# saga0619/libdwbc

Hardware: AMD Instinct MI355X
Metric: HQP control cycles/sec (batched TOCABI) (higher is better)
Workload: dtype f64; 1 GPU; BASELINE configs[1]: batch=1024 per GPU, TOCABI double support, 2-level HQP (pelvis 6D + upper-body rotation), tau limit 300, fp64; batch_per_gpu=1024, threads_per_instance=128, lds_bytes_per_instance=39152, collective_backend=none (one rank)

## Files before the change

__graft_entry__.py:

```python
import os
import subprocess
import sys

ROOT = os.path.dirname(os.path.abspath(__file__))
if ROOT not in sys.path:
    sys.path.insert(0, ROOT)


def build():
    env = dict(os.environ)
    env.setdefault("PYTORCH_ROCM_ARCH", "gfx950")
    csrc = os.path.join(ROOT, "libdwbc_amd", "csrc")
    import signal

    packs = [subprocess.Popen(["make", "-C", csrc, "pack", f"N={n}", f"NB={nb}", "ARCH=gfx950"], env=env, start_new_session=True)
             for n, nb in ((37, 32), (23, 18), (43, 38))]
    done = False
    try:
        subprocess.check_call(["make", "-C", csrc, "ARCH=gfx950"], env=env)
        subprocess.check_call(["make", "-C", os.path.join(ROOT, "oracle")], env=env)
        subprocess.check_call(["make", "-C", os.path.join(ROOT, "tests", "qp_probe"), "gpu", "ARCH=gfx950"], env=env)
        subprocess.check_call(["make", "-C", os.path.join(ROOT, "tests", "wave_probe"), "gpu", "ARCH=gfx950"], env=env)
        import libdwbc_amd
        from libdwbc_amd import _lib

        _lib.load()
        import tempfile

        from tests import cases

        with tempfile.TemporaryDirectory() as tmp:
            libdwbc_amd.build_pack(libdwbc_amd.Model.from_urdf(cases.variant_urdf(os.path.join(tmp, "fh.urdf"), cases.HEAD_JOINTS)), tree=True)
        for p in packs:
            if p.wait() != 0:
                raise subprocess.CalledProcessError(p.returncode, p.args)
        done = True
    finally:
        if not done:
            for p in packs:
                if p.poll() is None:
                    try:
                        os.killpg(p.pid, signal.SIGTERM)
                    except ProcessLookupError:
                        pass
            for p in packs:
                try:
                    p.wait(timeout=30)
                except subprocess.TimeoutExpired:
                    try:
                        os.killpg(p.pid, signal.SIGKILL)
                    except ProcessLookupError:
                        pass
                    p.wait()


def smoke():
    import numpy as np

    import libdwbc_amd as D
    from oracle import orc
    from tests import cases

    B = 16
    model = D.Model.from_urdf(cases.URDF)
    wbc = D.Batch(model, B, device=0)
    for c in cases.CONTACTS_2:
        wbc.add_contact(c["link"], c["point"], c["lx"], c["ly"], c["mu"], c["muz"])
    wbc.add_task(0, D.TASK_LINK_6D, 0)
    wbc.add_task(1, D.TASK_LINK_ROTATION, 15)
    wbc.set_torque_limit(np.array(cases.TAU_LIM))
    q, flags, fstar = cases.synth_batch(B, seed=7)
    wbc.set_state(q)
    wbc.set_contact(flags)
    wbc.set_fstar_all(fstar)
    wbc.solve()
    tau = wbc.get("tau")
    status = wbc.get("status")
    M = orc.make_model(cases.tocabi_model())
    S = orc.make_setup(cases.CONTACTS_2, cases.TASKS_2LEVEL, cases.TAU_LIM)
    tau_ref, wr_ref, st_ref, _ = orc.cycle_batch(M, S, q, flags, fstar, 1)
    err = float(np.abs(tau - tau_ref).max())
    assert (status == st_ref).all(), (status, st_ref)
    assert err < 1e-6, err
    print(f"smoke ok: B={B} max|tau - oracle| = {err:.3e}")


if __name__ == "__main__":
    build()
    if len(sys.argv) > 1 and sys.argv[1] == "smoke":
        smoke()
```

libdwbc_amd/csrc/dwbc_cycle2p.h:

```cpp
#pragma once
#include "dwbc_cycle2.h"

namespace dwbc {

template <int N, int NB, int NLV>
struct Lds4 {
    static constexpr bool compact = true;
    static constexpr bool batch_reads = true;
    static constexpr int M = N - 6;
    static constexpr int C = 6 * kMaxActiveContacts;
    static constexpr int K = C - 6;
    static constexpr int T = kMaxTaskDof;
    static constexpr int WLD = 32;
    static constexpr int max2(int a, int b) { return a > b ? a : b; }
    static constexpr int ev(int a) { return (a + 1) & ~1; }
    static constexpr int tg = 0;
    static constexpr int tt = tg + M;
    static constexpr int tc = tt + M;
    static constexpr int PC = tc + M;
    static constexpr int Rc = PC + C;
    static constexpr int Pc = Rc + kMaxActiveContacts * 9;
    static constexpr int fs = Pc + kMaxActiveContacts * 3;
    static constexpr int flg = fs + kMaxLevels * kMaxTaskDof;
    static constexpr int q = ev(flg + 4);
// ... 24 lines not shown
    static constexpr int c_Vb = Jtt + max2(NLV * N * T, C * N);
    static constexpr int c_VG = c_Vb + M * K;
    static constexpr int hs = c_VG + M * K;
    static constexpr int hs_size = 4 * 36 + 72;
    static constexpr int ms = hs + hs_size;
    static constexpr int c_s1 = ms;
    static constexpr int c_s2 = ms + max2(C * K, 64);
    static constexpr int c_Lam = c_s2;
    static constexpr int ms_size = max2(C * K, 64) + C * C;
    static constexpr int kin = ms + ms_size;
    static constexpr int k_Iw = kin;
    static constexpr int k_Ic = k_Iw + NB * 10;
    static constexpr int k_Rl = k_Iw + NB * 3;
    static constexpr int k_anc = k_Ic + NB * 10 - 2 * NB;
    static_assert(k_Rl + NB * 9 <= k_anc, "local rotations must not reach the ancestor indices");
    static constexpr int k_S = k_Ic + NB * 10;
    static constexpr int k_F = k_S + N * 6;
    static constexpr int kin_end = k_F + N * 6;
    static constexpr bool a_overlay = false, a_packed = true;
    static constexpr int k_A = U;
    static_assert(N * (N + 1) / 2 <= (UAend - U), "the staged mass matrix borrows the U / T1x-sized region");
    static constexpr int c_Y = kin;
    static constexpr int c_D = kin + C * N;
    static constexpr int c_BJ = c_D + (NLV * T + 1) * C;
    static constexpr int T1x = ev(max2(c_BJ + NLV * T * T, kin + 2 * T * M + 6 * T * T + 3 * T));
    static_assert(T1x + NLV * T * MS <= kin_end, "Y, D, the task Gram blocks and T1x borrow the phase-1a scratch");
    static constexpr int p4_dl = kin;
    static constexpr int p4_e = p4_dl + ev(NVS * C);
    static constexpr int p4_w = p4_e + C * VS;
    static constexpr int p4_ts = U;
    static constexpr int p4_cv = p4_ts + M * VS;
    static_assert(kin % 2 == 0 && U % 2 == 0, "16-byte aligned rows of the phase-4 blocks (lds_rows_axpy)");
    static_assert(p4_w + K * VS <= c_D, "phase-4 scratch stays below D and the task Gram blocks (the helper reads them in parallel)");
    static_assert(p4_cv + 6 * VS <= UAend, "torques and base residuals borrow the place of the staged mass matrix");
    static constexpr int c_QW = kin;
    static constexpr int c_QWp = c_QW + T * M;
    static constexpr int c_Pi = c_QWp + T * M;
    static constexpr int c_Z = c_Pi + T * T;
    static constexpr int c_s2b = c_Z + T * T;
    static constexpr int cod_Q = c_s2b + T * T, cod_v = cod_Q + T * T, cod_G = cod_v + 3 * T, cod_T = cod_G + T * T;
    static_assert(cod_T + T * T <= T1x, "slow-route scratch stays below T1x");
    static constexpr int xl(int lv) { return U; }
    static constexpr int t_base = Rw;
    static constexpr int wm = ev(t_base + NLV * 6);
    static constexpr int t_fv = wm + C * WLD;
    static constexpr int qp_V = t_fv + C;
    static constexpr int p5_end = qp_V + kQpLd;
    static_assert(p5_end <= fend, "QP scratch over the link frames");
    static constexpr int c_T1 = 0;
    static constexpr int total = kin_end;
    static constexpr int total_bytes = total * (int)sizeof(real_t) + 64;
    static constexpr int FNl = NwJw, comp = flg, Jcm = 0, Pt = 0, c_Gi = 0, T1r = T1x, c_Q = T1x, c_Jt = Jtt, t_F = wm, t_s1 = wm, jk = 0;
};

#if defined(DWBC_HOST_EMU)
#define DWBC_PAIR_BARRIER(i) ((void)0)
#elif defined(DWBC_STAGE_TIMERS)
#define DWBC_PAIR_BARRIER(i)                                                                      \
    do {                                                                                          \
        if (diag && th.tid == 0) diag[(is_main ? DG_TIME : DG_FTIME) + (i)] = (int)(clock64() - t_start_); \
        __syncthreads();                                                                          \
        if (diag && th.tid == 0 && is_main) diag[DG_FTIME + 8 + (i)] = (int)(clock64() - t_start_); \
    } while (0)
#else
#define DWBC_PAIR_BARRIER(i) __syncthreads()
#endif
#if defined(DWBC_HOST_EMU)
#define DWBC_PAIR_BARRIER_X() ((void)0)
#else
#define DWBC_PAIR_BARRIER_X() __syncthreads()
#endif
#if defined(DWBC_STAGE_TIMERS) && !defined(DWBC_HOST_EMU)
#define DWBC_PSTAMP(i) do { DWBC_SYNC(); if (diag && th.tid == 0) diag[DG_FTIME + (i)] = (int)(clock64() - t_start_); } while (0)
#ifndef DWBC_PMASK
#define DWBC_PMASK 0ull
#endif
#define DWBC_PSTAMP_M(i) do { if constexpr (((DWBC_PMASK) >> ((i) - 41)) & 1ull) DWBC_PSTAMP(i); } while (0)
#else
#define DWBC_PSTAMP(i) ((void)0)
#define DWBC_PSTAMP_M(i) ((void)0)
#endif

template <int MR, int NCV, int KV, bool SYNC_STORE, class FA, class FB, class FS, class FC>
DWBC_WDEV void wave_gemm(FA fa, FB fb, FS fstore, FC fc) {
    constexpr int MT = (MR + 15) / 16, KB = (KV + 3) / 4;
    static_assert(NCV <= 16, "one column tile");
#if !defined(DWBC_HOST_EMU)
    static_assert(sizeof(real_t) == 8, "fp64 build");
    typedef double g_d4 __attribute__((ext_vector_type(4)));
    const int lane = (int)(threadIdx.x & 63u), li = lane & 15, lk = lane >> 4;
    const int jc = (NCV < 16 && li >= NCV) ? NCV - 1 : li;
    double av[MT][KB], bv[KB];
    static_for<0, KB>([&](auto sc) {
        constexpr int s_ = decltype(sc)::value;
        constexpr bool kwhole = 4 * s_ + 3 < KV;
        const int kk = kwhole ? 4 * s_ + lk : (4 * s_ + lk < KV ? 4 * s_ + lk : KV - 1);
        const bool kin = kwhole || 4 * s_ + lk < KV;
        const double b_ = fb(sc, kk, jc);
        bv[s_] = kin ? b_ : 0.0;
        static_for<0, MT>([&](auto tc) {
            constexpr int t = decltype(tc)::value;
            constexpr bool rwhole = 16 * t + 15 < MR;
            const int ic = rwhole ? 16 * t + li : (16 * t + li < MR ? 16 * t + li : MR - 1);
            const double a_ = fa(tc, sc, ic, kk);
            av[t][s_] = kin ? a_ : 0.0;
        });
    });
    g_d4 acc[MT];
#pragma unroll
    for (int t = 0; t < MT; t++)
#pragma unroll
        for (int r = 0; r < 4; r++) {
            const int i = 16 * t + lk + 4 * r;
            acc[t][r] = fc(i < MR ? i : MR - 1, jc);
        }
#pragma unroll
    for (int s_ = 0; s_ < KB; s_++)
#pragma unroll
        for (int t = 0; t < MT; t++) acc[t] = __builtin_amdgcn_mfma_f64_16x16x4f64(av[t][s_], bv[s_], acc[t], 0, 0, 0);
    if (SYNC_STORE) DWBC_SYNC();
#pragma unroll
    for (int t = 0; t < MT; t++)
#pragma unroll
        for (int r = 0; r < 4; r++) {
            const int i = 16 * t + lk + 4 * r;
            if (i < MR && li < NCV) fstore(i, li, acc[t][r]);
        }
#else
    real_t tmp[MR][NCV];
    for (int i = 0; i < MR; i++)
        for (int j = 0; j < NCV; j++) tmp[i][j] = fc(i, j);
    static_for<0, KB>([&](auto sc) {
        constexpr int s_ = decltype(sc)::value;
        static_for<0, MT>([&](auto tc) {
            constexpr int t = decltype(tc)::value;
            for (int li = 0; li < 16; li++)
                for (int lk = 0; lk < 4; lk++) {
                    const int i = 16 * t + li, kk = 4 * s_ + lk;
                    if (i >= MR || kk >= KV) continue;
                    const real_t a_ = fa(tc, sc, i, kk);
                    for (int j = 0; j < NCV; j++) tmp[i][j] += a_ * fb(sc, kk, j);
                }
        });
    });
    for (int i = 0; i < MR; i++)
        for (int j = 0; j < NCV; j++) fstore(i, j, tmp[i][j]);
#endif
}
template <int MR, int NCV, int KV, bool SYNC_STORE, class FA, class FB, class FS>
DWBC_WDEV void wave_gemm(FA fa, FB fb, FS fstore) {
    wave_gemm<MR, NCV, KV, SYNC_STORE>(fa, fb, fstore, [](int, int) { return real_t(0.0); });
}

template <class R>
DWBC_WDEV int spd_inverse12_lds(R *Mx, R *Out, R *scl) {
#if defined(DWBC_HOST_EMU)
    return spd_inverse_small(Mx, 12, 12, Out, 12, scl);
#else
    static_assert(sizeof(R) == 8, "fp64 build");
    const int lane = (int)(threadIdx.x & 63u);
    DWBC_SYNC();
    double s[12], dg, dsc;
    {
        const int col = lane < 12 ? lane : 0;
        const double a = Mx[col * 12 + col];
        int e2 = 0;
        (void)frexp(a > 0.0 ? a : 1.0, &e2);
        dsc = (lane < 12 && a > 0.0) ? ldexp(1.0, -(e2 >> 1)) : 1.0;
        if (lane < 12) scl[lane] = dsc;
    }
    DWBC_SYNC();
    {
        const int col = lane < 12 ? lane : 0;
#pragma unroll
        for (int i = 0; i < 12; i++) {
            const double v_ = Mx[i * 12 + col] * scl[i] * dsc;
            s[i] = lane < 12 ? v_ : 0.0;
        }
        const double d_ = Mx[col * 12 + col] * dsc * dsc;
        dg = lane < 12 ? d_ : 1.0;
    }
    DWBC_SYNC();
    int ok = 1;
    {
        DWBC_LANE_OPAQUE(lp);
#pragma unroll
        for (int i = 0; i < 12; i++) s[i] = (i == lp) ? dg - 1.0 : s[i];
    }
    double dg2 = dg - 2.0;
    lds_pivot<12, 11, 0>(s, dg2, ok, (unsigned)(size_t)Mx, lane);
    ok = DWBC_FLAG_UNIFORM(ok);
    DWBC_SYNC();
    if (lane < 12) {
        DWBC_LANE_OPAQUE(le);
#pragma unroll
        for (int i = 0; i < 12; i++) {
            const double v_ = (i == le) ? -dg2 : -s[i];
            Out[i * 12 + lane] = v_ * scl[i] * dsc;
        }
    }
    DWBC_SYNC();
    return ok;
#endif
}

template <int N, int NB, int NLV, int NT, class Topo>
DWBC_DEV void cycle_instance_v2p(int wave, Thr th, const Setup &su, const BatchIO &io, int inst, real_t *L) {
    using S = Lds4<N, NB, NLV>;
    constexpr int M = S::M, C = S::C, T = S::T;
    constexpr bool kTree = !std::is_same<Topo, TopoGeneric>::value;
    static_assert(kTree, "the paired kernel is built for a constant kinematic tree");
    static_assert(kMaxActiveContacts == 2, "two 6D contacts");
    static_assert(N + 1 <= 64 && NB <= 64 && NT >= 1, "one q entry and one body per lane (request phase, *_lane forms of dwbc_front.h)");
    DWBC_LANE_DECL;
    const bool is_main = wave <= 0, is_help = wave != 0;
    const int nb = NB;
    const real_t *body = io.body;
    const int *topo = io.topo;
    const io_t *qin = io.q + (size_t)inst * (N + 1);
    int *diag = io.diag ? io.diag + (size_t)inst * DG_COUNT : nullptr;
    DWBC_STAMP_INIT();
    const int npair = topo[3 * nb];
    PLA(real_t, b_rec, kBodyStride);
    PL(int, b_par);
    PL(int, b_len);
    real_t q_base[7] = {0, 0, 0, 0, 0, 0, 0};
    PL(real_t, q_cp);
    PL(real_t, q_jt);
    LANES { LV(q_cp) = real_t(0.0); LV(q_jt) = real_t(0.0); LV(b_par) = 0; }
    int pairw[kCrbaPairRounds<N, NT>];
    if (is_main) {
        LANES {
            LV(q_cp) = (real_t)qin[lane < N + 1 ? lane : 0];
            LV(q_jt) = (real_t)qin[(lane >= 1 && lane < NB) ? 5 + lane : 0];
        }
        for (int a = 0; a < 6; a++) q_base[a] = (real_t)qin[a];
        q_base[6] = (real_t)qin[N];
        lane_record_fetch<NB, BF_RT, BF_MASS>(body, b_rec);
        LANES { LV(b_par) = topo[lane < NB ? lane : 0]; }
#pragma unroll
        for (int r = 0; r < kCrbaPairRounds<N, NT>; r++) pairw[r] = topo[3 * nb + 1 + (r * NT + th.tid < npair ? r * NT + th.tid : npair - 1)];
    }
    static_assert(kMaxLevels * kMaxTaskDof <= 64, "one f* entry per lane");
    PL(real_t, fs_req);
    LANES { LV(fs_req) = real_t(0.0); }
    if (is_help) {
        const io_t *fin = io.fstar + (size_t)inst * su.fstar_total;
        LANES {
            if (lane < su.fstar_total) LV(fs_req) = (real_t)fin[lane];
        }
    }
    const unsigned char *fl = io.flags + (size_t)inst * su.n_contacts;
    int flb[kMaxContacts];
    int lane_zero = 0;
    DWBC_FLAG_VGPR(lane_zero);
#pragma unroll
    for (int i = 0; i < kMaxContacts; i++) flb[i] = (i < su.n_contacts ? fl + i : (const unsigned char *)topo)[lane_zero];
    lane_record_fetch<NB, BF_MASS, kBodyStride>(body, b_rec);
    LANES { LV(b_len) = topo[2 * NB + (lane < NB ? lane : 0)]; }
    real_t *JCt = L + S::c_JC, *Yt = L + S::c_Y, *Lam = L + S::c_Lam, *JbT = L + S::JbT, *Vb = L + S::c_Vb, *VG = L + S::c_VG;
    real_t *flg = L + S::flg;

    PLA(real_t, s, N);
    PL(real_t, dg);
    int st_contact = 1;

    real_t *Rw = L + S::Rw, *pw = L + S::pw, *aw = L + S::aw, *Rl = L + S::k_Rl;
    real_t *Iw = L + S::k_Iw, *Icm = L + S::k_Ic, *Sm = L + S::k_S, *Fm = L + S::k_F;
    if (is_main) {
        LANES {
            if (lane < N + 1) L[S::q + lane] = LV(q_cp);
        }
        for (int i = th.tid; i < 3 * M; i += NT) L[S::tg + i] = real_t(0.0);
        DWBC_PSTAMP_M(56);
        constexpr int kRounds = jump_rounds(Topo::maxdepth);
        PLA(real_t, Ri, 9);
        PLA(real_t, pi, 3);
        PL(real_t, an);
        joint_transforms_lane<NB>(q_base, q_jt, b_rec, b_par, kRounds, Rw, pw, Rl, Iw, L + S::k_anc, Ri, pi, an);
        DWBC_PSTAMP_M(57);
        world_transforms_jump_lane<NB>(kRounds, Rw, pw, Rl, Iw, L + S::k_anc, Ri, pi, an);
        DWBC_PSTAMP_M(58);
        world_axes_lane<NB>(b_rec, Ri, aw);
        DWBC_PSTAMP_M(59);
    }
    if (is_help) {
        LANES {
            if (lane < su.fstar_total) L[S::fs + lane] = LV(fs_req);
        }
        if (th.tid == 0) { flg[0] = real_t(1.0); flg[1] = real_t(0.0); }
    }
    int act_c[kMaxActiveContacts] = {0, 0};
    int nc = 0, nflag = 0;
#pragma unroll
    for (int i = 0; i < kMaxContacts; i++) {
        if (i < su.n_contacts) {
            const int f_ = DWBC_FLAG_UNIFORM(flb[i]);
            if (f_ && nc < kMaxActiveContacts) act_c[nc++] = i;
            nflag += f_ ? 1 : 0;
        }
    }
    if (is_main) DWBC_PSTAMP_M(55);
    const bool too_many = nflag > kMaxActiveContacts;
    const int cd = 6 * nc, k = cd > 6 ? cd - 6 : 0;
    DWBC_PAIR_BARRIER(0);

    if (is_main) {
        world_inertias_lane<NB>(b_rec, Rw, pw, Iw);
        DWBC_SYNC();
        DWBC_PSTAMP_M(51);
        composite_inertias_scan_lane<0, 5>(b_len, nb, Iw, Icm);
        DWBC_SYNC();
    }
    if (is_help) {
        world_inertias_lane<NB>(b_rec, Rw, pw, Iw);
        DWBC_SYNC();
        composite_inertias_scan_lane<5, 10>(b_len, nb, Iw, Icm);
        DWBC_SYNC();
    }
    if (is_main) {
        motion_axes<N, NT>(th, Rw, pw, aw, Sm);
        DWBC_SYNC();
    }
    DWBC_PAIR_BARRIER_X();
    if (is_main) {
        DWBC_PSTAMP_M(52);
        body_forces<N, NT>(th, Icm, Sm, Fm);
        DWBC_SYNC();
        DWBC_PSTAMP_M(53);
        real_t *A = L + S::k_A;
        for (int idx = th.tid; idx < N * (N + 1) / 2; idx += NT) A[idx] = real_t(0.0);
        DWBC_SYNC();
        crba_pairs_fill<N, NT>(th, npair, pairw, Sm, Fm, A);
        DWBC_SYNC();
        DWBC_PSTAMP_M(54);
        load_mass_columns<N>(A, s, dg, L + S::G);
        DWBC_PSTAMP_M(41);
    }
    if (is_help) {
        for (int a = 0; a < nc; a++) {
            const int ci = act_c[a], link = su.c_link[ci];
            const real_t *R = Rw + link * 9;
            for (int r = th.tid; r < 12; r += NT) {
// ... 737 lines not shown
```

libdwbc_amd/csrc/dwbc_qp_wave.h:

```cpp
#pragma once
#include <type_traits>

#include "dwbc_wave.h"

namespace dwbc {

constexpr int kQpN = 12;

template <int QN>
struct QpRowsT {
    PLA(real_t, g, QN);
    PL(real_t, hi);
    PL(real_t, lo);
    PL(int, id_hi);
    PL(int, id_lo);
};
using QpRows = QpRowsT<kQpN>;

template <int QN>
struct QpResultT {
    int status, iters, nact;
    real_t viol;
    real_t x[QN];
    int act[QN];
#if defined(DWBC_STAGE_TIMERS) && !defined(DWBC_HOST_EMU)
    long long tm[10];
#endif
};
using QpResult = QpResultT<kQpN>;

#if defined(DWBC_STAGE_TIMERS) && !defined(DWBC_HOST_EMU)
#define DWBC_QPT_INIT() long long qpt_last_ = clock64(); for (int i_ = 0; i_ < 10; i_++) out.tm[i_] = 0
#define DWBC_QPT(i) do { const long long now_ = clock64(); out.tm[i] += now_ - qpt_last_; qpt_last_ = now_; } while (0)
#else
#define DWBC_QPT_INIT() ((void)0)
#define DWBC_QPT(i) ((void)0)
#endif

#ifdef DWBC_QP_TRACE
#ifdef DWBC_HOST_EMU
#define QP_TRACE(...) printf(__VA_ARGS__)
#else
#define QP_TRACE(...) do { if (threadIdx.x == 0) printf(__VA_ARGS__); } while (0)
#endif
#endif
#define DWBC_QP_INF (dwbc::kF32 ? dwbc::real_t(1.0e30) : dwbc::real_t(1.0e300))



template <int WS, int NV = kQpN, int QN = kQpN, int KCV = (QN > 12 ? QN - 6 : 6)>
DWBC_WDEV void qp_solve_wave(QpRowsT<QN> &R, int nv, int t, int max_iter, QpResultT<QN> &out, real_t *V , const int *warm,
                             real_t vtol, PL_REF(real_t, sfin)) {
    DWBC_LANE_DECL;
    static_assert(NV <= QN && NV <= 24, "variable count");
    constexpr int SB = NV > 16 ? 32 : 16;
    const int k = nv - t;
    PLA(real_t, Mx, NV);
    PL(real_t, d);
    PL(real_t, fs);
    PL(real_t, gnv);
    PL(real_t, u);
    PL(int, akey);
    PL(real_t, ehi);
    PL(real_t, elo);
    PL(bool, rok);
    PL(int, slotbit);
    PL(real_t, val);
    PL(int, key);
    PL(real_t, m);
    PL(real_t, dz);
    PL(real_t, xl);
    DWBC_QPT_INIT();
    LANES {
        LV(xl) = real_t(0.0);
        DWBC_LANE_OPAQUE(lq);
        real_t s2 = real_t(0.0), a2 = real_t(0.0);
#pragma unroll
        for (int j = 0; j < NV; j++) {
            const real_t g2 = LV(R.g)[j] * LV(R.g)[j];
            s2 += g2;
            a2 += (j < t) ? g2 : g2 * (real_t(1.0) / (kQpScaleGI * kQpScaleGI));
        }
        const bool zrow = s2 < kQpZeroRow * kQpZeroRow;
        const real_t gn = zrow ? real_t(1.0) : sqrt(s2);
        const real_t rg = zrow ? real_t(0.0) : real_t(1.0) / gn;
        LV(fs) = zrow ? real_t(1.0) : gn / sqrt(a2);
        LV(gnv) = gn;
#pragma unroll
        for (int j = 0; j < NV; j++) {
            LV(R.g)[j] *= rg;
            LV(Mx)[j] = (lq == j) ? real_t(1.0) : real_t(0.0);
        }
        if (LV(R.hi) < DWBC_QP_INF && !zrow) LV(R.hi) *= rg;
        if (LV(R.lo) < DWBC_QP_INF && !zrow) LV(R.lo) *= rg;
        LV(ehi) = LV(R.hi) >= DWBC_QP_INF ? DWBC_QP_INF : LV(R.hi);
        LV(elo) = LV(R.lo) >= DWBC_QP_INF ? DWBC_QP_INF : LV(R.lo);
        LV(d) = real_t(0.0);
        LV(u) = real_t(0.0);
        LV(akey) = 0;
        LV(slotbit) = (lane >= SB && lane < SB + NV) ? (1 << (lane - SB)) : 0;
        LV(m) = real_t(0.0);
        LV(dz) = real_t(0.0);
    }
    DWBC_QPT(6);
    int used = 0, q = 0, it = 0, status = 1, p = 0, side = 0, kmin = 0;
    bool pick = true;
    real_t up = real_t(0.0), worst = real_t(0.0);
    real_t sp = real_t(0.0);
    int wid[QN], wpos = QN;
    if (WS && warm) {
#pragma unroll
        for (int a = 0; a < QN; a++) wid[a] = warm[a];
        wpos = 0;
    }
    for (;;) {
        bool got = false;
        if (WS && pick) {
            while (wpos < QN && !got) {
                int id = -1;
#pragma unroll
                for (int a = 0; a < QN; a++) id = (a == wpos) ? wid[a] : id;
                wpos++;
                if (id < 0) continue;
                LANES {
                    const bool mh = LV(R.id_hi) == id && LV(ehi) < DWBC_QP_INF;
                    const bool ml = LV(R.id_lo) == id && LV(elo) < DWBC_QP_INF;
                    LV(val) = mh ? LV(ehi) - LV(d) : (ml ? LV(elo) + LV(d) : DWBC_QP_INF);
                    LV(key) = (lane << 1) | (ml ? 1 : 0);
                }
                int pl;
                WAVE_ARGMIN_F32(val, pl);
                worst = BCAST(val, pl);
                kmin = BCASTI(key, pl);
                if (worst < -vtol) got = true;
            }
            if (got) {
                p = kmin >> 1;
                side = kmin & 1;
                up = real_t(0.0);
                sp = worst;
                pick = false;
            }
        }
        if (pick) {
            LANES {
                const real_t sh = LV(ehi) - LV(d);
                const real_t sl = LV(elo) + LV(d);
                const bool lo_side = sl < sh;
                LV(val) = lo_side ? sl : sh;
                LV(key) = (lane << 1) | (lo_side ? 1 : 0);
            }
            int pl;
            WAVE_ARGMIN_F32(val, pl);
            worst = BCAST(val, pl);
            kmin = BCASTI(key, pl);
            DWBC_QPT(1);
            if (!(worst < -vtol)) break;
            p = kmin >> 1;
            side = kmin & 1;
            up = real_t(0.0);
            sp = worst;
            pick = false;
        }
        if (++it > max_iter) { status = 0; break; }
        real_t gp[NV];
#pragma unroll
        for (int j = 0; j < NV; j++) gp[j] = BCASTA(R.g, j, p);
        const real_t sgn = side ? real_t(1.0) : -real_t(1.0);
        LANES {
            real_t s_ = real_t(0.0);
#pragma unroll
            for (int j = 0; j < NV; j++) s_ += LV(Mx)[j] * gp[j];
            LV(m) = sgn * s_;
        }
        real_t zu[NV];
#pragma unroll
        for (int i = 0; i < NV; i++) zu[i] = BCAST(m, i);
        LANES {
            real_t s_ = real_t(0.0);
#pragma unroll
            for (int j = 0; j < NV; j++) s_ += LV(R.g)[j] * zu[j];
            LV(dz) = s_;
        }
        real_t zg = sgn * BCAST(dz, p);
        if (zg < kQpReorth) {
            LANES {
                real_t s_ = real_t(0.0);
#pragma unroll
                for (int j = 0; j < NV; j++) s_ += LV(Mx)[j] * zu[j];
                if (lane < NV) LV(m) = s_;
            }
#pragma unroll
            for (int i = 0; i < NV; i++) zu[i] = BCAST(m, i);
            LANES {
                real_t s_ = real_t(0.0);
#pragma unroll
                for (int j = 0; j < NV; j++) s_ += LV(R.g)[j] * zu[j];
                LV(dz) = s_;
            }
            zg = sgn * BCAST(dz, p);
        }
        const bool zok = zg > (kF32 ? real_t(1e-10) : real_t(1e-20)) && q < nv;
        DWBC_QPT(2);
        LANES { LV(rok) = (LV(slotbit) & used) && LV(m) > (kF32 ? real_t(1e-6) : real_t(1e-12)); }
        real_t t1 = DWBC_QP_INF;
        int l = SB;
        bool rany;
        WAVE_ANY(rok, rany);
        if (rany) {
            LANES {
                LV(val) = LV(rok) ? LV(u) * fast_rcp(LV(m)) : DWBC_QP_INF;
                LV(key) = lane;
            }
            if constexpr (SB == 16) {
                WAVE_ARGMIN_ROW1(val, key, t1, l);
            } else {
                WAVE_ARGMIN(val, key, t1, l);
            }
        }
        const real_t t2 = zok ? -sp * fast_rcp(zg) : DWBC_QP_INF;
        const real_t tstep = t1 < t2 ? t1 : t2;
        if (!(tstep < DWBC_QP_INF)) { status = 0; break; }
        const bool full = zok && t2 <= t1;
        if (zok) {
            LANES {
                LV(d) += tstep * LV(dz);
                LV(xl) += tstep * LV(m);
            }
        }
        LANES { LV(u) -= tstep * LV(m); }
        up += tstep;
        DWBC_QPT(3);
        if (full) {
            const int slot = __builtin_ctz(~(unsigned)used);
            const real_t inv_ = fast_rcp(zg);
            LANES {
                real_t coef = LV(m) * inv_;
                if (lane == SB + slot) { coef = -inv_; LV(u) = up; LV(akey) = kmin; }
#pragma unroll
                for (int j = 0; j < NV; j++) LV(Mx)[j] -= coef * zu[j];
                LV(ehi) = ((lane << 1) == kmin) ? DWBC_QP_INF : LV(ehi);
                LV(elo) = (((lane << 1) | 1) == kmin) ? DWBC_QP_INF : LV(elo);
            }
            used |= 1 << slot;
            q++;
            pick = true;
        } else {
            const int kl = BCASTI(akey, l);
            WSYNC();
            LANES {
                if (lane == l) {
#pragma unroll
                    for (int j = 0; j < NV; j++) V[j] = LV(Mx)[j];
                }
            }
            WSYNC();
            real_t rho[NV], rr = real_t(0.0);
#pragma unroll
            for (int j = 0; j < NV; j++) { rho[j] = V[j]; rr += rho[j] * rho[j]; }
            const real_t inv_ = fast_rcp(rr);
            LANES {
                real_t dd = real_t(0.0);
#pragma unroll
                for (int j = 0; j < NV; j++) dd += LV(Mx)[j] * rho[j];
                real_t coef = dd * inv_;
                if (lane < NV) coef = -V[lane] * inv_;
#pragma unroll
                for (int j = 0; j < NV; j++) LV(Mx)[j] = (lane == l) ? real_t(0.0) : LV(Mx)[j] - coef * rho[j];
                if (lane == l) LV(u) = real_t(0.0);
                LV(ehi) = ((lane << 1) == kl) ? LV(R.hi) : LV(ehi);
                LV(elo) = (((lane << 1) | 1) == kl) ? LV(R.lo) : LV(elo);
            }
            WSYNC();
            used &= ~(1 << (l - SB));
            q--;
            LANES { LV(val) = side ? LV(R.lo) + LV(d) : LV(R.hi) - LV(d); }
            sp = BCAST(val, p);
        }
        DWBC_QPT(4);
    }
    DWBC_QPT(0);
    out.iters = it;
    out.nact = q;
    out.status = status;
    out.viol = worst >= DWBC_QP_INF ? real_t(0.0) : worst;
#pragma unroll
    for (int a = 0; a < QN; a++) {
        if (WS) {
            const int ka = BCASTI(akey, SB + a);
            const int ow = ka >> 1;
            const int idh = BCASTI(R.id_hi, ow), idl = BCASTI(R.id_lo, ow);
            out.act[a] = ((used >> a) & 1) ? ((ka & 1) ? idl : idh) : -1;
        } else {
            out.act[a] = -1;
        }
    }
#pragma unroll
    for (int i = 0; i < QN; i++) out.x[i] = real_t(0.0);
    auto final_slack = [&](int which) {
        LANES {
            const real_t gx = which == 0 ? real_t(0.0) : (which == 1 ? LV(d) : LV(dz));
            const real_t sh = LV(R.hi) >= DWBC_QP_INF ? DWBC_QP_INF : (LV(R.hi) - gx) * LV(gnv);
            const real_t sl = LV(R.lo) >= DWBC_QP_INF ? DWBC_QP_INF : (LV(R.lo) + gx) * LV(gnv);
            LV(sfin) = sl < sh ? sl : sh;
        }
    };
    if (!status || q == 0) { final_slack(0); return; }
    real_t xu[NV];
#pragma unroll
    for (int i = 0; i < NV; i++) xu[i] = BCAST(xl, i);
#pragma unroll
    for (int j = 0; j < QN; j++) out.x[j] = (j < nv) ? xu[j < NV ? j : 0] * ((j >= t) ? kQpScaleGI : real_t(1.0)) : real_t(0.0);
    if (!(k > 0 && t > 0)) { final_slack(1); return; }
    {
        real_t xs[NV];
        constexpr int KC = KCV;
        constexpr int kCgMax = KC > kQpRefine ? 4 * KC : kQpRefine;
        static_assert(NV >= KC, "variable blocks");
        bool settled = false;
        auto lex_point = [&](auto std_tag) {
            constexpr bool STD = decltype(std_tag)::value;
            real_t cx[KC], cr[KC], cp[KC], cb[KC];
#pragma unroll
            for (int i = 0; i < KC; i++) {
                real_t v = real_t(0.0);
                if constexpr (STD) {
                    v = xu[NV - KC + i];
                } else {
#pragma unroll
                    for (int j = 0; j < NV; j++) v = (j == t + i && i < k) ? xu[j] : v;
                }
                cb[i] = v;
                cx[i] = v;
            }
            auto hmul = [&](const real_t (&v)[KC]) {
                LANES {
                    real_t s_ = real_t(0.0);
                    if constexpr (STD) {
#pragma unroll
                        for (int i = 0; i < KC; i++) s_ += LV(Mx)[NV - KC + i] * v[i];
                    } else {
#pragma unroll
                        for (int j = 0; j < NV; j++) {
                            real_t vj = real_t(0.0);
#pragma unroll
                            for (int i = 0; i < KC; i++) vj = (j == t + i && i < k) ? v[i] : vj;
                            s_ += LV(Mx)[j] * vj;
                        }
                    }
                    LV(m) = s_;
                }
            };
            auto hcc = [&](int i) -> real_t {
                real_t h_;
                if constexpr (STD) h_ = BCAST(m, NV - KC + i);
                else h_ = (i < k) ? BCAST(m, t + i) : real_t(0.0);
                return h_;
            };
            hmul(cx);
            real_t rs = real_t(0.0), bn = real_t(0.0);
#pragma unroll
            for (int i = 0; i < KC; i++) {
                cr[i] = cb[i] - (cx[i] - hcc(i));
                cp[i] = cr[i];
                rs += cr[i] * cr[i];
                bn += cb[i] * cb[i];
            }
            const real_t rtol2 = kQpRefineTol * kQpRefineTol * bn;
            bool nulldir = false;
            const real_t atol2 = kQpNullRes * kQpNullRes * bn;
            for (int r = 0; r < kCgMax && rs > rtol2; r++) {
#ifdef DWBC_QP_TRACE
                QP_TRACE("  cg %d rs %.3e\n", r, (double)rs);
#endif
                hmul(cp);
                real_t ap[KC], pap = real_t(0.0), pp = real_t(0.0);
#pragma unroll
                for (int i = 0; i < KC; i++) {
                    ap[i] = cp[i] - hcc(i);
                    pap += cp[i] * ap[i];
                    pp += cp[i] * cp[i];
                }
                if (!(pap > kQpNullDir * pp)) { nulldir = true; break; }
                const real_t al = rs * fast_rcp(pap);
                real_t rs2 = real_t(0.0);
#pragma unroll
                for (int i = 0; i < KC; i++) {
                    const real_t rn = cr[i] - al * ap[i];
                    rs2 += rn * rn;
                }
                if (rs2 > rs && !(rs > atol2)) { nulldir = true; break; }
#pragma unroll
                for (int i = 0; i < KC; i++) {
                    cx[i] += al * cp[i];
                    cr[i] -= al * ap[i];
                }
// ... 58 lines not shown
```

libdwbc_amd/csrc/dwbc_wave.h:

```cpp
#pragma once
#include <math.h>

#include "dwbc_types.h"

#ifdef DWBC_HOST_EMU
#define PL(type, x) type x[64]
#define PLA(type, x, n) type x[64][n]
#define LV(x) x[lane]
#define LANES for (int lane = 0; lane < 64; ++lane)
#define WSYNC() ((void)0)
#define DWBC_LANE_DECL ((void)0)
#define DWBC_LANE_OPAQUE(name) const int name = lane
#define DWBC_LANE_OPAQUE_IF(name, cond) const int name = lane
#define DWBC_FLAG_VGPR(f) ((void)0)
#define DWBC_FLAG_UNIFORM(f) (f)
#define BCAST(x, src) ((x)[(src)])
#define BCASTA(x, j, src) ((x)[(src)][(j)])
#define SHFLA(x, j, src) ((x)[(src)][(j)])
#define SHFL(x, src) ((x)[(src)])
#define DWBC_WDEV inline
#define PLA_REF(type, name, n) type (&name)[64][n]
#define PL_REF(type, name) type (&name)[64]
#else
#define PL(type, x) type x
// ... 149 lines not shown
    do {                                                                                           \
        out_b = false;                                                                             \
        for (int l_ = 0; l_ < 64; l_++) out_b = out_b || (flag)[l_];                               \
    } while (0)
#define WAVE_ARGMIN_ROW1(val, key, out_v, out_k)                                                   \
    do {                                                                                           \
        out_v = (val)[16];                                                                         \
        out_k = (key)[16];                                                                         \
        for (int l_ = 17; l_ < 32; l_++)                                                           \
            if ((val)[l_] < out_v || ((val)[l_] == out_v && (key)[l_] < out_k)) { out_v = (val)[l_]; out_k = (key)[l_]; } \
    } while (0)
#else
namespace dwbc {
__device__ __forceinline__ unsigned long long wave_min_u64(unsigned long long x) {
#define DWBC_DPP_STEP(ctrl, rmask)                                                                         \
    {                                                                                                      \
        const int lo_ = (int)(unsigned)(x & 0xffffffffull), hi_ = (int)(unsigned)(x >> 32);                \
        const int olo_ = __builtin_amdgcn_update_dpp(lo_, lo_, ctrl, rmask, 0xf, false);                   \
        const int ohi_ = __builtin_amdgcn_update_dpp(hi_, hi_, ctrl, rmask, 0xf, false);                   \
        const unsigned long long o_ = ((unsigned long long)(unsigned)ohi_ << 32) | (unsigned)olo_;         \
        x = o_ < x ? o_ : x;                                                                               \
    }
    DWBC_DPP_STEP(0x111, 0xf)
    DWBC_DPP_STEP(0x112, 0xf)
    DWBC_DPP_STEP(0x114, 0xf)
    DWBC_DPP_STEP(0x118, 0xf)
    DWBC_DPP_STEP(0x142, 0xa)
    DWBC_DPP_STEP(0x143, 0xc)
#undef DWBC_DPP_STEP
    const int lo = __builtin_amdgcn_readlane((int)(unsigned)(x & 0xffffffffull), 63);
    const int hi = __builtin_amdgcn_readlane((int)(unsigned)(x >> 32), 63);
    return ((unsigned long long)(unsigned)hi << 32) | (unsigned)lo;
}
__device__ __forceinline__ unsigned long long row1_min_u64(unsigned long long x) {
#define DWBC_DPP_STEP(ctrl)                                                                                \
    {                                                                                                      \
        const int lo_ = (int)(unsigned)(x & 0xffffffffull), hi_ = (int)(unsigned)(x >> 32);                \
        const int olo_ = __builtin_amdgcn_update_dpp(lo_, lo_, ctrl, 0xf, 0xf, false);                     \
        const int ohi_ = __builtin_amdgcn_update_dpp(hi_, hi_, ctrl, 0xf, 0xf, false);                     \
        const unsigned long long o_ = ((unsigned long long)(unsigned)ohi_ << 32) | (unsigned)olo_;         \
        x = o_ < x ? o_ : x;                                                                               \
    }
    DWBC_DPP_STEP(0x111)
    DWBC_DPP_STEP(0x112)
    DWBC_DPP_STEP(0x114)
    DWBC_DPP_STEP(0x118)
#undef DWBC_DPP_STEP
    const int lo = __builtin_amdgcn_readlane((int)(unsigned)(x & 0xffffffffull), 31);
    const int hi = __builtin_amdgcn_readlane((int)(unsigned)(x >> 32), 31);
    return ((unsigned long long)(unsigned)hi << 32) | (unsigned)lo;
}
__device__ __forceinline__ int wave_argmin_f32(real_t v) {
    const float f = (float)v;
    float m = f;
#define DWBC_DPP_STEP(ctrl, rmask)                                                                         \
    {                                                                                                      \
        const int o_ = __builtin_amdgcn_update_dpp(__float_as_int(m), __float_as_int(m), ctrl, rmask, 0xf, false); \
        m = fminf(m, __int_as_float(o_));                                                                  \
    }
    DWBC_DPP_STEP(0x111, 0xf)
    DWBC_DPP_STEP(0x112, 0xf)
    DWBC_DPP_STEP(0x114, 0xf)
    DWBC_DPP_STEP(0x118, 0xf)
    DWBC_DPP_STEP(0x142, 0xa)
    DWBC_DPP_STEP(0x143, 0xc)
#undef DWBC_DPP_STEP
    const float mall = __int_as_float(__builtin_amdgcn_readlane(__float_as_int(m), 63));
    const unsigned long long b = __ballot(f == mall);
    return b ? (int)__builtin_ctzll(b) : 0;
}
__device__ __forceinline__ double wave_sum_f64(double x) {
#define DWBC_DPP_STEP(ctrl, rmask)                                                                         \
    {                                                                                                      \
        const long long b_ = __double_as_longlong(x);                                                      \
        const int lo_ = (int)(unsigned)(b_ & 0xffffffffll), hi_ = (int)(unsigned)((unsigned long long)b_ >> 32); \
        const int olo_ = __builtin_amdgcn_update_dpp(0, lo_, ctrl, rmask, 0xf, true);                      \
        const int ohi_ = __builtin_amdgcn_update_dpp(0, hi_, ctrl, rmask, 0xf, true);                      \
        x += __longlong_as_double((long long)(((unsigned long long)(unsigned)ohi_ << 32) | (unsigned)olo_)); \
    }
    DWBC_DPP_STEP(0x111, 0xf)
    DWBC_DPP_STEP(0x112, 0xf)
    DWBC_DPP_STEP(0x114, 0xf)
    DWBC_DPP_STEP(0x118, 0xf)
    DWBC_DPP_STEP(0x142, 0xa)
    DWBC_DPP_STEP(0x143, 0xc)
#undef DWBC_DPP_STEP
    return readlane_f64(x, 63);
}
__device__ __forceinline__ double wave_prefix_f64(double x) {
#define DWBC_DPP_STEP(ctrl, rmask)                                                                         \
    {                                                                                                      \
        const long long b_ = __double_as_longlong(x);                                                      \
        const int lo_ = (int)(unsigned)(b_ & 0xffffffffll), hi_ = (int)(unsigned)((unsigned long long)b_ >> 32); \
        const int olo_ = __builtin_amdgcn_update_dpp(0, lo_, ctrl, rmask, 0xf, true);                      \
        const int ohi_ = __builtin_amdgcn_update_dpp(0, hi_, ctrl, rmask, 0xf, true);                      \
        x += __longlong_as_double((long long)(((unsigned long long)(unsigned)ohi_ << 32) | (unsigned)olo_)); \
    }
    DWBC_DPP_STEP(0x111, 0xf)
    DWBC_DPP_STEP(0x112, 0xf)
    DWBC_DPP_STEP(0x114, 0xf)
    DWBC_DPP_STEP(0x118, 0xf)
    DWBC_DPP_STEP(0x142, 0xa)
    DWBC_DPP_STEP(0x143, 0xc)
#undef DWBC_DPP_STEP
    return x;
}
__device__ __forceinline__ float wave_prefix_f64(float x) {
#define DWBC_DPP_STEP(ctrl, rmask) x += __int_as_float(__builtin_amdgcn_update_dpp(0, __float_as_int(x), ctrl, rmask, 0xf, true));
    DWBC_DPP_STEP(0x111, 0xf)
    DWBC_DPP_STEP(0x112, 0xf)
    DWBC_DPP_STEP(0x114, 0xf)
    DWBC_DPP_STEP(0x118, 0xf)
    DWBC_DPP_STEP(0x142, 0xa)
    DWBC_DPP_STEP(0x143, 0xc)
#undef DWBC_DPP_STEP
    return x;
}
__device__ __forceinline__ float wave_sum_f64(float x) {
#define DWBC_DPP_STEP(ctrl, rmask) x += __int_as_float(__builtin_amdgcn_update_dpp(0, __float_as_int(x), ctrl, rmask, 0xf, true));
    DWBC_DPP_STEP(0x111, 0xf)
    DWBC_DPP_STEP(0x112, 0xf)
    DWBC_DPP_STEP(0x114, 0xf)
    DWBC_DPP_STEP(0x118, 0xf)
    DWBC_DPP_STEP(0x142, 0xa)
    DWBC_DPP_STEP(0x143, 0xc)
#undef DWBC_DPP_STEP
    return readlane_f64(x, 63);
}
__device__ __forceinline__ unsigned long long argmin_key(real_t v, int lane) {
    unsigned long long b = (unsigned long long)__double_as_longlong((double)v);
    b = (b >> 63) ? ~b : (b | 0x8000000000000000ull);
    return (b & ~127ull) | (unsigned)lane;
}
}
#define WAVE_ARGMIN(val, key, out_v, out_k)                                                        \
    do {                                                                                           \
        const unsigned long long m_ = dwbc::wave_min_u64(dwbc::argmin_key((val), lane));           \
        const int wl_ = (int)(m_ & 127ull);                                                        \
        out_v = dwbc::readlane_f64((val), wl_);                                                    \
        out_k = dwbc::readlane_i32((key), wl_);                                                    \
    } while (0)
#define WAVE_ARGMIN_F32(val, out_lane) out_lane = dwbc::wave_argmin_f32(val)
#define WAVE_ANY(flag, out_b) out_b = __ballot(flag) != 0ull
#define WAVE_SUM(val, out_v) out_v = dwbc::wave_sum_f64(val)
#define WAVE_PREFIX_A(arr, j) (arr)[(j)] = dwbc::wave_prefix_f64((arr)[(j)])
#define WAVE_ARGMIN_ROW1(val, key, out_v, out_k)                                                   \
    do {                                                                                           \
        const unsigned long long m_ = dwbc::row1_min_u64(dwbc::argmin_key((val), lane));           \
        const int wl_ = (int)(m_ & 127ull);                                                        \
        out_v = dwbc::readlane_f64((val), wl_);                                                    \
        out_k = dwbc::readlane_i32((key), wl_);                                                    \
    } while (0)
#endif
```

Before: 19.55 million cycles/s.

## Use DPP row_newbcast FMA chains for QP and 12x12 inverse pivots

Replaces the per-element lane broadcasts (readlane or LDS) in the wave QP's dz/Mx updates and in the 12x12 SPD inverse pivot loop with inline-asm v_fmac_f64_dpp row_newbcast chains. Row 0 is first replicated across all four DPP rows with permlane16/32 swaps. This is meant to remove the scalar broadcast and LDS round-trip latency in these inner loops. It relies on gfx950-specific DPP and permlane instructions, hand-placed s_nop hazards, and the assumption that NV is at most 16.

```diff
diff --git a/__graft_entry__.py b/__graft_entry__.py
--- a/__graft_entry__.py
+++ b/__graft_entry__.py
@@ -21,6 +21,7 @@
         subprocess.check_call(["make", "-C", os.path.join(ROOT, "oracle")], env=env)
         subprocess.check_call(["make", "-C", os.path.join(ROOT, "tests", "qp_probe"), "gpu", "ARCH=gfx950"], env=env)
         subprocess.check_call(["make", "-C", os.path.join(ROOT, "tests", "wave_probe"), "gpu", "ARCH=gfx950"], env=env)
+        subprocess.check_call(["make", "-C", os.path.join(ROOT, "tests", "rowbc_probe"), "gpu", "ARCH=gfx950"], env=env)
         import libdwbc_amd
         from libdwbc_amd import _lib
 
diff --git a/libdwbc_amd/csrc/dwbc_cycle2p.h b/libdwbc_amd/csrc/dwbc_cycle2p.h
--- a/libdwbc_amd/csrc/dwbc_cycle2p.h
+++ b/libdwbc_amd/csrc/dwbc_cycle2p.h
@@ -200,6 +200,23 @@
     wave_gemm<MR, NCV, KV, SYNC_STORE>(fa, fb, fstore, [](int, int) { return real_t(0.0); });
 }
 
+#if !defined(DWBC_HOST_EMU)
+template <int K>
+__device__ __forceinline__ void rowbc_pivot12(double (&s)[12], double &dg2, int &ok, int lane) {
+    double d = readlane_f64(dg2, K) + 2.0;
+    int pos = d > 0.0 ? 1 : 0;
+    DWBC_FLAG_VGPR(pos);
+    ok &= pos;
+    if (!(d > 0.0)) d = 1.0;
+    const double rp = fast_rcp(d);
+    const double cj = s[K];
+    const double h = cj * rp;
+    rowbc_axpy<12>(s, cj, -h);
+    dg2 = (lane == K) ? -rp : dg2 - cj * h;
+    if constexpr (K > 0) rowbc_pivot12<K - 1>(s, dg2, ok, lane);
+}
+#endif
+
 template <class R>
 DWBC_WDEV int spd_inverse12_lds(R *Mx, R *Out, R *scl) {
 #if defined(DWBC_HOST_EMU)
@@ -236,7 +253,7 @@
         for (int i = 0; i < 12; i++) s[i] = (i == lp) ? dg - 1.0 : s[i];
     }
     double dg2 = dg - 2.0;
-    lds_pivot<12, 11, 0>(s, dg2, ok, (unsigned)(size_t)Mx, lane);
+    rowbc_pivot12<11>(s, dg2, ok, lane);
     ok = DWBC_FLAG_UNIFORM(ok);
     DWBC_SYNC();
     if (lane < 12) {
diff --git a/libdwbc_amd/csrc/dwbc_qp_wave.h b/libdwbc_amd/csrc/dwbc_qp_wave.h
--- a/libdwbc_amd/csrc/dwbc_qp_wave.h
+++ b/libdwbc_amd/csrc/dwbc_qp_wave.h
@@ -55,6 +55,7 @@
     static_assert(NV <= QN && NV <= 24, "variable count");
     constexpr int SB = NV > 16 ? 32 : 16;
     const int k = nv - t;
+    constexpr bool kRowBc = !kF32 && NV <= 16;
     PLA(real_t, Mx, NV);
     PL(real_t, d);
     PL(real_t, fs);
@@ -174,29 +175,49 @@
             LV(m) = sgn * s_;
         }
         real_t zu[NV];
-#pragma unroll
-        for (int i = 0; i < NV; i++) zu[i] = BCAST(m, i);
-        LANES {
-            real_t s_ = real_t(0.0);
-#pragma unroll
-            for (int j = 0; j < NV; j++) s_ += LV(R.g)[j] * zu[j];
-            LV(dz) = s_;
+        PL(real_t, mz);
+        if constexpr (kRowBc) {
+            LANES { LV(mz) = LV(m); LV(dz) = real_t(0.0); }
+            ROW_REPLICATE(mz);
+            ROWBC_DOT(NV, dz, mz, R.g);
+        } else {
+#pragma unroll
+            for (int i = 0; i < NV; i++) zu[i] = BCAST(m, i);
+            LANES {
+                real_t s_ = real_t(0.0);
+#pragma unroll
+                for (int j = 0; j < NV; j++) s_ += LV(R.g)[j] * zu[j];
+                LV(dz) = s_;
+            }
         }
         real_t zg = sgn * BCAST(dz, p);
         if (zg < kQpReorth) {
-            LANES {
-                real_t s_ = real_t(0.0);
-#pragma unroll
-                for (int j = 0; j < NV; j++) s_ += LV(Mx)[j] * zu[j];
-                if (lane < NV) LV(m) = s_;
-            }
-#pragma unroll
-            for (int i = 0; i < NV; i++) zu[i] = BCAST(m, i);
-            LANES {
-                real_t s_ = real_t(0.0);
-#pragma unroll
-                for (int j = 0; j < NV; j++) s_ += LV(R.g)[j] * zu[j];
-                LV(dz) = s_;
+            if constexpr (kRowBc) {
+                PL(real_t, hz);
+                LANES { LV(hz) = real_t(0.0); }
+                ROWBC_DOT(NV, hz, mz, Mx);
+                LANES {
+                    if (lane < NV) LV(m) = LV(hz);
+                    LV(mz) = LV(m);
+                    LV(dz) = real_t(0.0);
+                }
+                ROW_REPLICATE(mz);
+                ROWBC_DOT(NV, dz, mz, R.g);
+            } else {
+                LANES {
+                    real_t s_ = real_t(0.0);
+#pragma unroll
+                    for (int j = 0; j < NV; j++) s_ += LV(Mx)[j] * zu[j];
+                    if (lane < NV) LV(m) = s_;
+                }
+#pragma unroll
+                for (int i = 0; i < NV; i++) zu[i] = BCAST(m, i);
+                LANES {
+                    real_t s_ = real_t(0.0);
+#pragma unroll
+                    for (int j = 0; j < NV; j++) s_ += LV(R.g)[j] * zu[j];
+                    LV(dz) = s_;
+                }
             }
             zg = sgn * BCAST(dz, p);
         }
@@ -234,14 +255,20 @@
         if (full) {
             const int slot = __builtin_ctz(~(unsigned)used);
             const real_t inv_ = fast_rcp(zg);
+            PL(real_t, ncoef);
             LANES {
                 real_t coef = LV(m) * inv_;
                 if (lane == SB + slot) { coef = -inv_; LV(u) = up; LV(akey) = kmin; }
-#pragma unroll
-                for (int j = 0; j < NV; j++) LV(Mx)[j] -= coef * zu[j];
+                if constexpr (kRowBc) {
+                    LV(ncoef) = -coef;
+                } else {
+#pragma unroll
+                    for (int j = 0; j < NV; j++) LV(Mx)[j] -= coef * zu[j];
+                }
                 LV(ehi) = ((lane << 1) == kmin) ? DWBC_QP_INF : LV(ehi);
                 LV(elo) = (((lane << 1) | 1) == kmin) ? DWBC_QP_INF : LV(elo);
             }
+            if constexpr (kRowBc) ROWBC_AXPY(NV, Mx, mz, ncoef);
             used |= 1 << slot;
             q++;
             pick = true;
diff --git a/libdwbc_amd/csrc/dwbc_wave.h b/libdwbc_amd/csrc/dwbc_wave.h
--- a/libdwbc_amd/csrc/dwbc_wave.h
+++ b/libdwbc_amd/csrc/dwbc_wave.h
@@ -325,3 +325,83 @@
         out_k = dwbc::readlane_i32((key), wl_);                                                    \
     } while (0)
 #endif
+
+#ifdef DWBC_HOST_EMU
+#define ROWBC_FMA(J, acc, x, y)                                                                                        \
+    do {                                                                                                               \
+        for (int l_ = 0; l_ < 64; l_++) (acc)[l_] += (x)[(l_ & ~15) | (J)] * (y)[l_];          \
+    } while (0)
+#define ROWBC_DOT(N, acc, x, y)                                                                                        \
+    do {                                                                                                               \
+        for (int l_ = 0; l_ < 64; l_++)                                                                                \
+            for (int j_ = 0; j_ < (N); j_++) (acc)[l_] += (x)[(l_ & ~15) | j_] * (y)[l_][j_];  \
+    } while (0)
+#define ROWBC_AXPY(N, a, x, c)                                                                                         \
+    do {                                                                                                               \
+        for (int l_ = 0; l_ < 64; l_++)                                                                                \
+            for (int j_ = 0; j_ < (N); j_++) (a)[l_][j_] += (x)[(l_ & ~15) | j_] * (c)[l_];  \
+    } while (0)
+#define ROW_REPLICATE(x)                                                                                               \
+    do {                                                                                                               \
+        for (int l_ = 16; l_ < 64; l_++) (x)[l_] = (x)[l_ & 15];                                                       \
+    } while (0)
+#else
+namespace dwbc {
+#define DWBC_RB_DOT_(j, y) "v_fmac_f64_dpp %0, %1, %" #y " row_newbcast:" #j " row_mask:0xf bank_mask:0xf\n"
+#define DWBC_RB_AXPY_(j, x, c) "v_fmac_f64_dpp %" #j ", %" #x ", %" #c " row_newbcast:" #j " row_mask:0xf bank_mask:0xf\n"
+template <int J>
+__device__ __forceinline__ void rowbc_fma(double &acc, double x, double y) {
+    static_assert(J >= 0 && J < 16, "a lane of the own DPP row");
+    asm volatile("s_nop 1\nv_fmac_f64_dpp %0, %1, %2 row_newbcast:%3 row_mask:0xf bank_mask:0xf" : "+&v"(acc) : "v"(x), "v"(y), "n"(J));
+}
+template <int N, int NY>
+__device__ __forceinline__ void rowbc_dot(double &acc, double x, const double (&y)[NY]) {
+    static_assert((N == 6 || N == 9 || N == 12) && N <= NY, "chain lengths of the wave QP");
+    if constexpr (N == 6)
+        asm volatile("s_nop 1\n" DWBC_RB_DOT_(0, 2) DWBC_RB_DOT_(1, 3) DWBC_RB_DOT_(2, 4) DWBC_RB_DOT_(3, 5) DWBC_RB_DOT_(4, 6) DWBC_RB_DOT_(5, 7)
+                     : "+&v"(acc) : "v"(x), "v"(y[0]), "v"(y[1]), "v"(y[2]), "v"(y[3]), "v"(y[4]), "v"(y[5]));
+    if constexpr (N == 9)
+        asm volatile("s_nop 1\n" DWBC_RB_DOT_(0, 2) DWBC_RB_DOT_(1, 3) DWBC_RB_DOT_(2, 4) DWBC_RB_DOT_(3, 5) DWBC_RB_DOT_(4, 6) DWBC_RB_DOT_(5, 7)
+                     DWBC_RB_DOT_(6, 8) DWBC_RB_DOT_(7, 9) DWBC_RB_DOT_(8, 10)
+                     : "+&v"(acc) : "v"(x), "v"(y[0]), "v"(y[1]), "v"(y[2]), "v"(y[3]), "v"(y[4]), "v"(y[5]), "v"(y[6]), "v"(y[7]), "v"(y[8]));
+    if constexpr (N == 12)
+        asm volatile("s_nop 1\n" DWBC_RB_DOT_(0, 2) DWBC_RB_DOT_(1, 3) DWBC_RB_DOT_(2, 4) DWBC_RB_DOT_(3, 5) DWBC_RB_DOT_(4, 6) DWBC_RB_DOT_(5, 7)
+                     DWBC_RB_DOT_(6, 8) DWBC_RB_DOT_(7, 9) DWBC_RB_DOT_(8, 10) DWBC_RB_DOT_(9, 11) DWBC_RB_DOT_(10, 12) DWBC_RB_DOT_(11, 13)
+                     : "+&v"(acc) : "v"(x), "v"(y[0]), "v"(y[1]), "v"(y[2]), "v"(y[3]), "v"(y[4]), "v"(y[5]), "v"(y[6]), "v"(y[7]), "v"(y[8]), "v"(y[9]),
+                       "v"(y[10]), "v"(y[11]));
+}
+template <int N, int NA>
+__device__ __forceinline__ void rowbc_axpy(double (&a)[NA], double x, double c) {
+    static_assert((N == 6 || N == 9 || N == 12) && N <= NA, "chain lengths of the wave QP");
+    if constexpr (N == 6)
+        asm volatile("s_nop 1\n" DWBC_RB_AXPY_(0, 6, 7) DWBC_RB_AXPY_(1, 6, 7) DWBC_RB_AXPY_(2, 6, 7) DWBC_RB_AXPY_(3, 6, 7) DWBC_RB_AXPY_(4, 6, 7)
+                     DWBC_RB_AXPY_(5, 6, 7)
+                     : "+&v"(a[0]), "+&v"(a[1]), "+&v"(a[2]), "+&v"(a[3]), "+&v"(a[4]), "+&v"(a[5]) : "v"(x), "v"(c));
+    if constexpr (N == 9)
+        asm volatile("s_nop 1\n" DWBC_RB_AXPY_(0, 9, 10) DWBC_RB_AXPY_(1, 9, 10) DWBC_RB_AXPY_(2, 9, 10) DWBC_RB_AXPY_(3, 9, 10) DWBC_RB_AXPY_(4, 9, 10)
+                     DWBC_RB_AXPY_(5, 9, 10) DWBC_RB_AXPY_(6, 9, 10) DWBC_RB_AXPY_(7, 9, 10) DWBC_RB_AXPY_(8, 9, 10)
+                     : "+&v"(a[0]), "+&v"(a[1]), "+&v"(a[2]), "+&v"(a[3]), "+&v"(a[4]), "+&v"(a[5]), "+&v"(a[6]), "+&v"(a[7]), "+&v"(a[8]) : "v"(x), "v"(c));
+    if constexpr (N == 12)
+        asm volatile("s_nop 1\n" DWBC_RB_AXPY_(0, 12, 13) DWBC_RB_AXPY_(1, 12, 13) DWBC_RB_AXPY_(2, 12, 13) DWBC_RB_AXPY_(3, 12, 13)
+                     DWBC_RB_AXPY_(4, 12, 13) DWBC_RB_AXPY_(5, 12, 13) DWBC_RB_AXPY_(6, 12, 13) DWBC_RB_AXPY_(7, 12, 13) DWBC_RB_AXPY_(8, 12, 13)
+                     DWBC_RB_AXPY_(9, 12, 13) DWBC_RB_AXPY_(10, 12, 13) DWBC_RB_AXPY_(11, 12, 13)
+                     : "+&v"(a[0]), "+&v"(a[1]), "+&v"(a[2]), "+&v"(a[3]), "+&v"(a[4]), "+&v"(a[5]), "+&v"(a[6]), "+&v"(a[7]), "+&v"(a[8]), "+&v"(a[9]),
+                       "+&v"(a[10]), "+&v"(a[11])
+                     : "v"(x), "v"(c));
+}
+#undef DWBC_RB_DOT_
+#undef DWBC_RB_AXPY_
+__device__ __forceinline__ double row_replicate(double x) {
+    const unsigned lo = (unsigned)__double2loint(x), hi = (unsigned)__double2hiint(x);
+    const auto l16 = __builtin_amdgcn_permlane16_swap(lo, lo, false, false);
+    const auto h16 = __builtin_amdgcn_permlane16_swap(hi, hi, false, false);
+    const auto l32 = __builtin_amdgcn_permlane32_swap(l16[0], l16[0], false, false);
+    const auto h32 = __builtin_amdgcn_permlane32_swap(h16[0], h16[0], false, false);
+    return __hiloint2double((int)h32[0], (int)l32[0]);
+}
+}
+#define ROWBC_FMA(J, acc, x, y) dwbc::rowbc_fma<J>((acc), (x), (y))
+#define ROWBC_DOT(N, acc, x, y) dwbc::rowbc_dot<N>((acc), (x), (y))
+#define ROWBC_AXPY(N, a, x, c) dwbc::rowbc_axpy<N>((a), (x), (c))
+#define ROW_REPLICATE(x) (x) = dwbc::row_replicate(x)
+#endif
```

New measurement: 19.77 million cycles/s (median of 6 runs). 1.1% higher.
